# erget/libaec

Measured on AMD Instinct MI355X. Metric: encode+decode GB/s (input bytes), higher is better.
Workload: dtype u32; 1 GPU; c2: lowent16 4096 MiB per GPU, 16-bit, block 16, rsi 128, flags 8; step = encode + decode (segment table); block_size=16, rsi=128, flags=8, input_bytes_per_gpu=4294967296, compressed_bytes_rank0=763194472, parallelism=1 independent shard stream(s)

## Files before the change

libaec_amd/csrc/aec_dec.hip:

```cpp
#include <hip/hip_runtime.h>

#include <cstdio>
#include <cstdlib>
#include <mutex>
#include <type_traits>

#include "aec_kernels.h"
#include "aec_lane.h"
#include "aec_spec.h"
#include "aec_tune.h"

namespace aec {

struct SegSum {
    int64_t sum, lo, hi;
    uint64_t end;
    uint32_t ref;
    uint32_t ok;
};

struct BareArgs {
    SegSum *sums = nullptr;
    const uint32_t *list = nullptr, *list_cnt = nullptr;
    uint64_t avg_hint = 0;
};

struct DecLaunch {
    const Cfg *c = nullptr;
    const uint32_t *words = nullptr;
    uint64_t nwords = 0, end_bit = 0;
    const uint64_t *rsi_off = nullptr;
    const SegEntry *seg_table = nullptr;
    uint64_t n_items = 0, total_blocks = 0;
    uint8_t *out = nullptr;
    DecResult *res = nullptr;
    hipStream_t st = nullptr;
    uint8_t *dump = nullptr;
    const DecResult *idx = nullptr, *batch = nullptr;
    uint32_t rpc = 0;
    bool win = false;
    bool next_entry = false;
    uint32_t rpc_arg() const { return win ? (next_entry ? 1u : 0u) : rpc; }
    BareArgs ba;
};
template <int BS> void dec_part_bytes(bool seg, bool sums, const DecLaunch &a);
template <int BS> void dec_part_wave(const DecLaunch &a);

namespace {

__device__ __forceinline__ uint32_t wave_incl_sum_dpp(uint32_t v)
{
    v += __builtin_amdgcn_update_dpp(0u, v, 0x111, 0xf, 0xf, false);
    v += __builtin_amdgcn_update_dpp(0u, v, 0x112, 0xf, 0xf, false);
    v += __builtin_amdgcn_update_dpp(0u, v, 0x114, 0xf, 0xf, false);
    v += __builtin_amdgcn_update_dpp(0u, v, 0x118, 0xf, 0xf, false);
    v += __builtin_amdgcn_update_dpp(0u, v, 0x142, 0xa, 0xf, false);
    v += __builtin_amdgcn_update_dpp(0u, v, 0x143, 0xc, 0xf, false);
    return v;
}

template <int BS, int BYTES>
__device__ __forceinline__ void store_block(uint8_t *dst, const uint32_t *d, const Cfg &c, bool ref,
                                            uint32_t &x)
{
    const bool pp = c.flags & F_PREPROCESS, sgn = c.flags & F_SIGNED, msb = c.flags & F_MSB;
    uint32_t v[BS];
    if (!pp) {
#pragma unroll
        for (int i = 0; i < BS; i++) v[i] = d[i];
    } else {
        const uint32_t x0 = ref ? (sgn ? sign_extend(d[0], c.bps) : d[0]) : x;
        const uint32_t d0 = ref ? 0u : d[0];
        uint32_t sum = d0, any = 0;
#pragma unroll
        for (int i = 1; i + 1 < BS; i += 2) sum += d[i] + d[i + 1];
        if (BS % 2 == 0) sum += d[BS - 1];
        if (BYTES == 4) {
#pragma unroll
            for (int i = 0; i < BS; i++) any |= i == 0 ? d0 : d[i];
        }
        const uint32_t below = sgn ? x0 + c.xmax + 1u : x0, above = c.xmax - x0;
        const bool fits = sum <= below && sum <= above && (BYTES != 4 || (any >> 26) == 0u);
        if (!__any(!fits)) {
            uint32_t xx = x0;
#pragma unroll
            for (int i = 0; i < BS; i++) {
                const uint32_t di = i == 0 ? d0 : d[i];
                xx += (di >> 1) ^ (uint32_t)__builtin_amdgcn_sbfe((int)di, 0u, 1u);
                v[i] = xx;
            }
            x = xx;
        } else {
#pragma unroll
            for (int i = 0; i < BS; i++) {
                if (i == 0 && ref) {
                    x = x0;
                } else {
                    x = sgn ? unpp_signed(x, d[i], c.xmax) : unpp_unsigned(x, d[i], c.xmax);
                }
                v[i] = x;
            }
        }
    }
    if (BYTES == 4) {
        uint4 *o = reinterpret_cast<uint4 *>(dst);
#pragma unroll
        for (int q = 0; q < BS / 4; q++) {
            uint32_t w[4];
#pragma unroll
            for (int j = 0; j < 4; j++) w[j] = msb ? bswap32(v[4 * q + j]) : v[4 * q + j];
            o[q] = make_uint4(w[0], w[1], w[2], w[3]);
        }
    } else if (BYTES == 2) {
        const uint32_t sel = msb ? 0x04050001u : 0x05040100u;
        uint32_t w[BS / 2];
#pragma unroll
        for (int j = 0; j < BS / 2; j++) w[j] = __builtin_amdgcn_perm(v[2 * j + 1], v[2 * j], sel);
        if (BS >= 8) {
            uint4 *o = reinterpret_cast<uint4 *>(dst);
#pragma unroll
            for (int q = 0; q < BS / 8; q++) o[q] = make_uint4(w[4 * q], w[4 * q + 1], w[4 * q + 2], w[4 * q + 3]);
        }
    } else if (BYTES == 1) {
        uint32_t w[BS / 4];
#pragma unroll
        for (int j = 0; j < BS / 4; j++)
            w[j] = __builtin_amdgcn_perm(v[4 * j + 1], v[4 * j], 0x0c0c0400u) |
                   __builtin_amdgcn_perm(v[4 * j + 3], v[4 * j + 2], 0x04000c0cu);
        uint2 *o = reinterpret_cast<uint2 *>(dst);
#pragma unroll
        for (int q = 0; q < BS / 8; q++) o[q] = make_uint2(w[2 * q], w[2 * q + 1]);
    } else {
#pragma unroll
        for (int i = 0; i < BS; i++) {
            const uint32_t s = v[i];
            dst[3 * i + 0] = (uint8_t)(msb ? s >> 16 : s);
            dst[3 * i + 1] = (uint8_t)(s >> 8);
            dst[3 * i + 2] = (uint8_t)(msb ? s : s >> 16);
        }
    }
}

__device__ __forceinline__ void store_block_generic(uint8_t *dst, const uint32_t *d, const Cfg &c, bool ref,
                                                    uint32_t &x)
{
    const bool pp = c.flags & F_PREPROCESS, sgn = c.flags & F_SIGNED, msb = c.flags & F_MSB;
    for (uint32_t i = 0; i < c.bs; i++) {
        uint32_t v;
        if (!pp) v = d[i];
        else if (i == 0 && ref) v = x = sgn ? sign_extend(d[0], c.bps) : d[0];
        else v = x = sgn ? unpp_signed(x, d[i], c.xmax) : unpp_unsigned(x, d[i], c.xmax);
        for (uint32_t t = 0; t < c.bytes; t++)
            dst[i * c.bytes + t] = (uint8_t)(v >> (8 * (msb ? c.bytes - 1 - t : t)));
    }
}

__device__ __forceinline__ void report(DecResult *res, uint32_t status, uint64_t rsi, uint64_t block)
{
    atomicMax(&res->status, status);
    atomicMin(reinterpret_cast<unsigned long long *>(&res->bad_rsi), (unsigned long long)rsi);
    atomicMin(reinterpret_cast<unsigned long long *>(&res->tail_blocks), (unsigned long long)block);
}

template <bool SEG>
__device__ __forceinline__ void dec_counts(const Cfg &c, const DecResult *idx, uint64_t &n_items, uint64_t &total_blocks)
{
    if (!idx) return;
    const uint64_t whole = idx->n_rsi, tail = idx->tail_blocks;
    n_items = whole + (tail ? 1u : 0u);
    total_blocks = whole * c.rsi + tail;
    if (SEG) n_items *= c.segs_per_rsi;
}

struct DecItem {
    uint32_t nb;
    uint64_t start, first_blk;
};
__device__ __forceinline__ DecItem dec_item(const Cfg &c, uint64_t r, uint64_t total_blocks, const uint64_t *__restrict__ rsi_off,
                                            const DecResult *__restrict__ batch, uint32_t rsi_per_chunk)
{
    DecItem it;
    if (batch) {
        const uint64_t sidx = r / rsi_per_chunk;
        const uint32_t rin = (uint32_t)(r - sidx * rsi_per_chunk);
        const uint64_t whole = batch[sidx].n_rsi, tail = batch[sidx].tail_blocks;
        it.nb = rin < whole ? c.rsi : (rin == whole ? (uint32_t)tail : 0u);
        it.start = it.nb ? rsi_off[r] : 0;
    } else {
        const uint64_t left = total_blocks - r * c.rsi;
        it.nb = left > c.rsi ? c.rsi : (uint32_t)left;
        it.start = rsi_off[r];
    }
    it.first_blk = r * c.rsi;
    return it;
}

__device__ __forceinline__ void report_item(DecResult *res, const DecResult *batch, uint32_t rsi_per_chunk, uint32_t status,
                                            uint64_t r, uint64_t block)
{
    report(res, status, r, block);
    if (batch && status == DEC_DATA_ERROR)
        atomicMax(&const_cast<DecResult *>(batch)[r / rsi_per_chunk].status, (uint32_t)DEC_DATA_ERROR);
}

__device__ __forceinline__ void win_end_check(const Cfg &c, DecResult *res, const uint64_t *__restrict__ rsi_off, uint64_t r,
                                              uint64_t n_rsi, uint32_t next_entry, uint64_t end, uint64_t last_blk)
{
    if (r + 1u < n_rsi + next_entry) {
        const uint64_t e = (c.flags & F_PAD_RSI) ? (end + 7u) & ~7ull : end;
        if (e != rsi_off[r + 1u]) report(res, DEC_DATA_ERROR, r, last_blk);
    }
}

struct RingSrc {
    const uint32_t *col;
    uint32_t slot0, mask;
    uint32_t limit;
    uint32_t starve;
    __device__ __forceinline__ uint32_t word(uint32_t i)
    {
        starve |= (i >= limit) ? 1u : 0u;
        return col[((slot0 + i) & mask) * 64u];
    }
    __device__ __forceinline__ void word2(uint32_t i, uint32_t &w0, uint32_t &w1)
    {
        starve |= (i + 1 >= limit) ? 1u : 0u;
        const uint32_t *q = col + ((slot0 + i) & mask) * 64u;
        w0 = q[0];
        w1 = q[64];
    }
    __device__ __forceinline__ void word3(uint32_t i, uint32_t &w0, uint32_t &w1, uint32_t &w2)
    {
        starve |= (i + 2 >= limit) ? 1u : 0u;
        const uint32_t *q = col + ((slot0 + i) & mask) * 64u;
        w0 = q[0];
        w1 = q[64];
        w2 = q[128];
    }
    __device__ __forceinline__ bool starved() const { return starve != 0; }
};

__device__ __forceinline__ uint4 load_words4(const uint32_t *__restrict__ words, uint64_t idx, uint64_t nwords)
{
    uint4 v = make_uint4(0, 0, 0, 0);
    if (idx + 4 <= nwords) {
        v = *reinterpret_cast<const uint4 *>(words + idx);
    } else {
        if (idx < nwords) v.x = words[idx];
        if (idx + 1 < nwords) v.y = words[idx + 1];
        if (idx + 2 < nwords) v.z = words[idx + 2];
    }
    return v;
}

__device__ __forceinline__ uint4 load_words4_nb(const uint32_t *__restrict__ words, uint64_t idx, uint64_t last_chunk)
{
    if (idx > last_chunk) idx = last_chunk;
    return *reinterpret_cast<const uint4 *>(words + idx);
}

__device__ __forceinline__ void ring_put4(uint32_t *col, uint32_t slot0, uint32_t mask, uint32_t rel, uint4 v)
{
    const uint32_t row = (slot0 + rel) & mask;
    uint32_t *q = col + row * 64u;
    const uint32_t x = bswap32(v.x), y = bswap32(v.y);
    q[0] = x;
    q[64] = y;
    q[128] = bswap32(v.z);
    q[192] = bswap32(v.w);
    if (row == 0) {
        col[(mask + 1u) * 64u] = x;
        col[(mask + 2u) * 64u] = y;
    }
}

template <int BYTES>
struct SumAcc {
    typedef int64_t type;
    static constexpr int64_t kLo = -((int64_t)1 << 60), kHi = (int64_t)1 << 60;
};
template <>
struct SumAcc<1> {
    typedef int32_t type;
    static constexpr int32_t kLo = -(1 << 30), kHi = 1 << 30;
};
template <>
struct SumAcc<2> {
    typedef int32_t type;
    static constexpr int32_t kLo = -(1 << 30), kHi = 1 << 30;
};

template <int BS, typename ACC>
__device__ __forceinline__ void seg_accumulate(const uint32_t *d, bool first_is_ref, ACC R, ACC &P, ACC &lo, ACC &hi)
{
#pragma unroll
    for (int i = 0; i < BS; i++) {
        const uint32_t v = (i == 0 && first_is_ref) ? 0u : d[i];
        const ACC h = (ACC)((v >> 1) + (v & 1u));
        const ACC step = (v & 1u) ? -h : h;
        const ACC nlo = h - P, nhi = R - h - P;
        lo = nlo > lo ? nlo : lo;
        hi = nhi < hi ? nhi : hi;
        P += step;
    }
}

#ifndef AEC_STG_ROW
#define AEC_STG_ROW 64
#endif
#ifndef AEC_STG_ROW8
#define AEC_STG_ROW8 32
#endif
#ifndef AEC_DEC_MINW
#define AEC_DEC_MINW 1
#endif
#ifndef AEC_DEC_UNR8
#define AEC_DEC_UNR8 2
#endif
#ifndef AEC_DEC_OU
#define AEC_DEC_OU 1
#endif
#ifndef AEC_DEC_UNR16
#define AEC_DEC_UNR16 1
#endif
__host__ __device__ constexpr uint32_t dec_unroll(int bs) { return bs == 8 ? AEC_DEC_UNR8 : (bs == 16 ? AEC_DEC_UNR16 : 1); }
__host__ __device__ constexpr bool stg_on(int blk) { return blk == 16 || blk == 32 || (blk == 8 && AEC_STG_ROW8 != 0); }
__host__ __device__ constexpr uint32_t stg_row(int blk) { return blk == 8 ? (AEC_STG_ROW8 ? AEC_STG_ROW8 : 64) : AEC_STG_ROW; }

template <int BS, int BYTES, bool SEG, int kPend, bool SUMS = false, bool WIN = false>
__global__ void __launch_bounds__(256, AEC_DEC_MINW)
k_decode(const Cfg c, const uint32_t *__restrict__ words, uint64_t nwords, uint64_t end_bit,
         const uint64_t *__restrict__ rsi_off, const SegEntry *__restrict__ seg_table, uint64_t n_rsi,
         uint64_t total_blocks, uint8_t *__restrict__ out, DecResult *res, uint32_t ring_words, uint32_t maxw,
         uint32_t needw, uint8_t *__restrict__ dump, const DecResult *__restrict__ idx,
         const DecResult *__restrict__ batch, uint32_t rsi_per_chunk, SegSum *__restrict__ sums,
         const uint32_t *__restrict__ list, const uint32_t *__restrict__ list_cnt)
{
    static_assert(!SUMS || (SEG && BS != 0), "the summing pass runs per segment on the templated block sizes");
    static_assert(!WIN || (!SEG && !SUMS), "windows are tables of RSI starts");
    if (idx) {
        const uint64_t whole = idx->n_rsi, tail = idx->tail_blocks;
        n_rsi = whole + (tail ? 1u : 0u);
        total_blocks = whole * c.rsi + tail;
        if (SEG) n_rsi *= c.segs_per_rsi;
    }
    extern __shared__ __attribute__((aligned(16))) uint32_t smem[];
    const uint32_t lane = threadIdx.x & 63u, wave = threadIdx.x >> 6;
    const uint64_t nwords_vec = nwords >= 4 ? ((nwords + 3) & ~3ull) - 4 : 0;
    constexpr int BLK = BS * BYTES;
    constexpr bool STG = !SUMS && stg_on(BLK);
    constexpr uint32_t kStgRow = stg_row(BLK), kStgStride = kStgRow + 16u;
    constexpr uint32_t G = STG ? kStgRow / (uint32_t)(BLK ? BLK : 1) : 1u;
    const uint32_t wave_words = (ring_words + 2u) * 64u + (STG ? (64u * kStgStride) / 4u : 0u);
    uint32_t *wbase = smem + (size_t)wave * wave_words;
    uint32_t *col = wbase + lane;
    uint8_t *stage = reinterpret_cast<uint8_t *>(wbase + (ring_words + 2u) * 64u);
    const uint32_t mask = ring_words - 1;

    uint64_t r = ((uint64_t)blockIdx.x * (blockDim.x >> 6) + wave) * 64u + lane;
    bool active = r < n_rsi;
    if (!SEG && list) {
        active = r < *list_cnt;
        r = active ? list[r] : 0u;
    }
    constexpr int DN = BS ? BS : (int)kMaxBlockSize;
    const uint32_t bs = BS ? (uint32_t)BS : c.bs;
    const bool pp = c.flags & F_PREPROCESS;

    uint32_t nb = 0, b0 = 0, x = 0;
    uint64_t start = 0, first_blk = 0;
    if (active) {
        if (SEG) {
            const uint64_t rsi_idx = (r >> 32) ? r / c.segs_per_rsi : (uint64_t)((uint32_t)r / c.segs_per_rsi);
            b0 = (uint32_t)(r - rsi_idx * c.segs_per_rsi) * 64u;
            uint64_t left = total_blocks > rsi_idx * c.rsi ? total_blocks - rsi_idx * c.rsi : 0u;
            if (left > c.rsi) left = c.rsi;
            nb = left <= b0 ? 0u : (left - b0 > 64 ? 64u : (uint32_t)(left - b0));
            if (SUMS) {
                start = rsi_off[r];
            } else {
                const SegEntry e = seg_table[r];
                start = e.bit;
                x = (c.flags & F_SIGNED) ? sign_extend(e.prev, c.bps) : e.prev;
            }
            if (start == ~0ull) {
                start = 0;
                nb = 0;
            }
            first_blk = rsi_idx * c.rsi + b0;
        } else if (batch) {
            const uint64_t sidx = r / rsi_per_chunk;
            const uint32_t rin = (uint32_t)(r - sidx * rsi_per_chunk);
            const uint64_t whole = batch[sidx].n_rsi, tail = batch[sidx].tail_blocks;
            nb = rin < whole ? c.rsi : (rin == whole ? (uint32_t)tail : 0u);
            start = nb ? rsi_off[r] : 0;
            first_blk = r * c.rsi;
        } else {
            uint64_t left = total_blocks - r * c.rsi;
            nb = left > c.rsi ? c.rsi : (uint32_t)left;
            start = rsi_off[r];
            first_blk = r * c.rsi;
        }
    }
    const size_t blk_bytes = (size_t)bs * c.bytes;
    uint8_t *dst = out + (size_t)first_blk * blk_bytes;
    const uint32_t dst_lo = (uint32_t)reinterpret_cast<uintptr_t>(dst), dst_hi = (uint32_t)(reinterpret_cast<uintptr_t>(dst) >> 32);
    uint32_t produced = 0;
    auto flush = [&](uint32_t group) {
        const uint32_t filled = produced * (uint32_t)BLK;
        produced = 0;
        constexpr uint32_t LPR = kStgRow / 16u, RPI = 64u / LPR;
#pragma unroll
        for (uint32_t k = 0; k < LPR; k++) {
            const uint32_t row = k * RPI + lane / LPR, chunk = (lane % LPR) * 16u;
            const uint4 v = *reinterpret_cast<const uint4 *>(stage + row * kStgStride + chunk);
            const uint32_t have = __shfl(filled, (int)row);
            const uintptr_t rbase = (uintptr_t)__shfl(dst_lo, (int)row) | ((uintptr_t)__shfl(dst_hi, (int)row) << 32);
            uint8_t *at = reinterpret_cast<uint8_t *>(rbase) + (size_t)group * kStgRow + chunk;
            uint8_t *q = chunk + 16u <= have ? at : dump + (size_t)lane * 16u;
            typedef uint32_t u32x4 __attribute__((ext_vector_type(4)));
            typedef __attribute__((address_space(1))) u32x4 global_u32x4;
            const u32x4 vv = {v.x, v.y, v.z, v.w};
            if (kStgRow >= 64u)
                __builtin_nontemporal_store(vv, reinterpret_cast<global_u32x4 *>(reinterpret_cast<uintptr_t>(q)));
            else
                *reinterpret_cast<global_u32x4 *>(reinterpret_cast<uintptr_t>(q)) = vv;
            if (BLK == 8) {
                const bool half = have == chunk + 8u;
                if (__any(half)) {
                    typedef uint32_t u32x2 __attribute__((ext_vector_type(2)));
                    typedef __attribute__((address_space(1))) u32x2 global_u32x2;
                    const u32x2 hv = {v.x, v.y};
                    if (half) *reinterpret_cast<global_u32x2 *>(reinterpret_cast<uintptr_t>(at)) = hv;
                }
            }
        }
    };

    const uint64_t a0 = (start >> 5) & ~3ull;
    const uint32_t slot0 = (uint32_t)a0 & mask;
    uint32_t landed = 0;
    for (; landed < ring_words; landed += 4)
        ring_put4(col, slot0, mask, landed, load_words4(words, a0 + landed, nwords));

    RingSrc src{col, slot0, mask, landed, 0u};
    const uint64_t left_bits = end_bit - a0 * 32u;
    const uint32_t end_p = left_bits > 0xFFFFFFF0ull ? 0xFFFFFFF0u : (uint32_t)left_bits;
    uint32_t p = (uint32_t)(start - a0 * 32u);
    WinReader<RingSrc> br;
    if (BS == 0) br.init(src, a0 * 32u, end_bit, p);

    uint4 pend[kPend];
    uint32_t pv[kPend];
#pragma unroll
    for (int j = 0; j < kPend; j++) { pend[j] = make_uint4(0, 0, 0, 0); pv[j] = 0u; }

    uint32_t d[DN];
    uint32_t zrun = 0;
    uint32_t ok = 1u;
    typedef typename SumAcc<BYTES>::type acc_t;
    const acc_t acc_R = (acc_t)(((uint64_t)1 << c.bps) - 1u);
    acc_t acc_P = 0, acc_lo = SumAcc<BYTES>::kLo, acc_hi = SumAcc<BYTES>::kHi;
    uint32_t sum_ref = 0, sum_bad = 0, sum_done = 0;

    constexpr uint32_t UNR = (STG && G % dec_unroll(BS) != 0) ? 1u : dec_unroll(BS);
    constexpr uint32_t OU = (STG && AEC_DEC_OU && G > UNR) ? G / UNR : 1u;
    static_assert(!STG || G % UNR == 0, "a staging row holds whole top-up groups");
    uint32_t b = 0;
    for (; __any(b < nb && ok); b += OU * UNR) {
#pragma unroll
      for (uint32_t ou = 0; ou < OU; ou++) {
        const uint32_t bo = b + ou * UNR;
        const bool live = bo < nb && ok;
        {
            const uint32_t next = BS ? (p >> 5) : br.next;
            if (__any(live && landed - next < needw)) {
#pragma unroll
                for (int j = 0; j < kPend; j++) {
                    if (pv[j]) {
                        ring_put4(col, slot0, mask, landed, pend[j]);
                        landed += 4;
                    }
                    pv[j] = 0u;
                }
                while (__any(live && landed - next < needw)) {
                    uint4 t[kPend];
#pragma unroll
                    for (int j = 0; j < kPend; j++) t[j] = load_words4(words, a0 + landed + 4u * j, nwords);
#pragma unroll
                    for (int j = 0; j < kPend; j++)
                        if (live && landed - next < needw && landed + 4u - next <= ring_words) {
                            ring_put4(col, slot0, mask, landed, t[j]);
                            landed += 4;
                        }
                }
            }
        }

        const uint32_t ref = (pp && b0 + bo == 0) ? 1u : 0u;
        if (BS) {
#pragma unroll
          for (uint32_t uu = 0; uu < UNR; uu++) {
            const uint32_t bb = bo + uu;
            const bool live = bb < nb && ok;
            const uint32_t ref = (pp && b0 + bb == 0) ? 1u : 0u;
            src.limit = landed;
            src.starve = 0u;
            uint32_t nz = 0;
            const bool parse = live && zrun == 0;
            const uint32_t p_save = p;
            uint32_t st;
#pragma nounroll
            for (uint32_t attempt = 0;; attempt++) {
                st = decode_block<(BS ? BS : 2)>(src, p, end_p, d, c, ref, b0 + bb, parse, nz);
                if (attempt != 0 || needw >= maxw || !__any(parse && src.starved())) break;
                const uint32_t first = p_save >> 5;
#pragma unroll
                for (int j = 0; j < kPend; j++) {
                    if (pv[j]) {
                        ring_put4(col, slot0, mask, landed, pend[j]);
                        landed += 4;
                    }
                    pv[j] = 0u;
                }
                while (__any(live && landed + 4u - first <= ring_words)) {
                    if (live && landed + 4u - first <= ring_words) {
                        ring_put4(col, slot0, mask, landed, load_words4(words, a0 + landed, nwords));
                        landed += 4;
                    }
                }
                src.limit = landed;
                src.starve = 0;
                p = p_save;
                nz = 0;
            }
            const bool over = parse && (((p + 31u) >> 5) > landed || (st != DEC_OK && src.starved()));
            if (SUMS) {
                if (parse && (over || st != DEC_OK)) {
                    sum_bad = 1u;
                    ok = 0u;
                } else if (parse && nz) {
                    zrun = nz;
                }
            } else if (over) {
                atomicOr(&res->pad, kDecRedo);
                ok = 0u;
            } else if (parse) {
                if (st != DEC_OK) {
                    report(res, st, SEG ? (first_blk + bb) / c.rsi : r, first_blk + bb);
                    if (batch && st == DEC_DATA_ERROR)
                        atomicMax(&const_cast<DecResult *>(batch)[r / rsi_per_chunk].status, (uint32_t)DEC_DATA_ERROR);
                    ok = 0u;
                } else if (nz) {
                    zrun = nz;
                }
            }
            if (uu == 0) {
#pragma unroll
                for (int j = 0; j < kPend; j++)
                    if (pv[j]) {
                        ring_put4(col, slot0, mask, landed, pend[j]);
                        landed += 4;
                    }
                const uint32_t next = p >> 5;
#pragma unroll
                for (int j = 0; j < kPend; j++) {
                    pv[j] = (live && ok && (landed + 4u * j + 4u - next <= ring_words)) ? 1u : 0u;
                    const uint64_t idx = pv[j] ? a0 + landed + 4u * j : 0;
                    pend[j] = load_words4_nb(words, idx, nwords_vec);
                }
            }
            if (SUMS) {
                const bool st_ok = live && ok;
                const bool rf = ref != 0 && parse;
                if (st_ok) {
                    if (rf) sum_ref = d[0];
                    if (c.flags & F_PREPROCESS) seg_accumulate<DN, acc_t>(d, rf, acc_R, acc_P, acc_lo, acc_hi);
                    sum_done++;
                }
                zrun -= (st_ok && zrun) ? 1u : 0u;
            } else if (STG) {
                const bool st_ok = live && ok;
                store_block<DN, (BYTES ? BYTES : 1)>(stage + lane * kStgStride + (bb % G) * (uint32_t)BLK, d, c,
                                                     ref != 0 && parse, x);
                produced += st_ok ? 1u : 0u;
                zrun -= (st_ok && zrun) ? 1u : 0u;
                if (OU * UNR == G ? (ou * UNR + uu == G - 1u) : ((bb % G) == G - 1u)) flush(bb / G);
            } else {
                const bool st_ok = live && ok;
                uint8_t *q = st_ok ? dst : dump + (size_t)lane * blk_bytes;
                store_block<DN, (BYTES ? BYTES : 1)>(q, d, c, ref != 0 && parse, x);
                dst += st_ok ? blk_bytes : 0;
                zrun -= (st_ok && zrun) ? 1u : 0u;
            }
          }
        } else if (live) {
            br.src.limit = landed;
            bool rf = ref != 0;
            if (zrun == 0) {
                uint32_t nz = 0;
                const uint32_t st = parse_cds<0>(br, d, c, ref, b0 + bo, nz);
                if (br.src.starved()) {
                    atomicOr(&res->pad, kDecRedo);
                    ok = 0u;
                } else if (st != DEC_OK) {
                    report(res, st, r, first_blk + bo);
                    if (batch && st == DEC_DATA_ERROR)
                        atomicMax(&const_cast<DecResult *>(batch)[r / rsi_per_chunk].status, (uint32_t)DEC_DATA_ERROR);
                    ok = 0u;
                } else if (nz) {
                    const uint32_t keep = d[0];
                    for (int i = 0; i < DN; i++) d[i] = 0;
                    if (rf) d[0] = keep;
                    zrun = nz - 1;
                }
            } else {
                zrun--;
                rf = false;
            }
            if (ok) {
                store_block_generic(dst, d, c, rf, x);
                dst += blk_bytes;
                if (rf) d[0] = 0;
            }
        }
    }
    }
    if (STG && (b % G) != 0) flush(b / G);
    if (SUMS) {
        if (active) {
            SegSum o;
            o.sum = (int64_t)acc_P;
            o.lo = (int64_t)acc_lo;
            o.hi = (int64_t)acc_hi;
            o.end = a0 * 32u + p;
            o.ref = sum_ref;
            o.ok = (nb != 0u && !sum_bad && sum_done == nb && zrun == 0u) ? 1u : 0u;
            sums[r] = o;
        }
        return;
    }
    if constexpr (WIN) {
        if (active && ok && nb == c.rsi && r + 1u < n_rsi + rsi_per_chunk) {
            uint64_t e;
            if constexpr (BS != 0) e = a0 * 32u + p;
            else e = br.pos();
            if (c.flags & F_PAD_RSI) e = (e + 7u) & ~7ull;
            if (e != rsi_off[r + 1u]) report(res, DEC_DATA_ERROR, r, first_blk + nb - 1u);
        }
    }
    if (!SEG && active && (list ? first_blk + nb == total_blocks : r + 1 == n_rsi)) res->end_bit = x;
    if (SEG && active && nb && first_blk + nb == total_blocks) res->end_bit = x;
}

template <bool SEG, bool WIN = false>
__global__ void __launch_bounds__(64)
k_decode_redo(const Cfg c, const uint32_t *__restrict__ words, uint64_t nwords, uint64_t end_bit,
              const uint64_t *__restrict__ rsi_off, const SegEntry *__restrict__ seg_table, uint64_t n_rsi,
              uint64_t total_blocks, uint8_t *__restrict__ out, DecResult *res, const DecResult *__restrict__ idx,
              const DecResult *__restrict__ batch, uint32_t rsi_per_chunk, const uint32_t *__restrict__ list,
              const uint32_t *__restrict__ list_cnt)
{
    if (!(*reinterpret_cast<volatile uint32_t *>(&res->pad) & kDecRedo)) return;
    dec_counts<SEG>(c, idx, n_rsi, total_blocks);
    if (!SEG && list) n_rsi = *list_cnt;
    const bool pp = c.flags & F_PREPROCESS;
    const size_t blk_bytes = (size_t)c.bs * c.bytes;
    for (uint64_t r_lin = (uint64_t)blockIdx.x * 64u + threadIdx.x; r_lin < n_rsi; r_lin += (uint64_t)gridDim.x * 64u) {
        const uint64_t r = (!SEG && list) ? list[r_lin] : r_lin;
        uint32_t nb = 0, b0 = 0, x = 0;
        uint64_t start = 0, first_blk = 0;
        if (SEG) {
            const uint64_t rsi_idx = r / c.segs_per_rsi;
            b0 = (uint32_t)(r - rsi_idx * c.segs_per_rsi) * 64u;
            uint64_t left = total_blocks > rsi_idx * c.rsi ? total_blocks - rsi_idx * c.rsi : 0u;
            if (left > c.rsi) left = c.rsi;
            nb = left <= b0 ? 0u : (left - b0 > 64 ? 64u : (uint32_t)(left - b0));
            const SegEntry e = seg_table[r];
            if (e.bit == ~0ull) continue;
            start = e.bit;
            x = (c.flags & F_SIGNED) ? sign_extend(e.prev, c.bps) : e.prev;
            first_blk = rsi_idx * c.rsi + b0;
        } else if (batch) {
            const uint64_t sidx = r / rsi_per_chunk;
            const uint32_t rin = (uint32_t)(r - sidx * rsi_per_chunk);
            const uint64_t whole = batch[sidx].n_rsi, tail = batch[sidx].tail_blocks;
            nb = rin < whole ? c.rsi : (rin == whole ? (uint32_t)tail : 0u);
            start = nb ? rsi_off[r] : 0;
            first_blk = r * c.rsi;
        } else {
            const uint64_t left = total_blocks - r * c.rsi;
            nb = left > c.rsi ? c.rsi : (uint32_t)left;
            start = rsi_off[r];
            first_blk = r * c.rsi;
        }
        uint8_t *dst = out + (size_t)first_blk * blk_bytes;
        BitReader br;
        br.init(words, nwords, end_bit, start);
        uint32_t d[kMaxBlockSize];
        uint32_t zrun = 0;
        bool whole = true;
        for (uint32_t bo = 0; bo < nb; bo++) {
            bool rf = pp && b0 + bo == 0;
            if (zrun == 0) {
                uint32_t nz = 0;
                const uint32_t st = parse_cds<0>(br, d, c, rf ? 1u : 0u, b0 + bo, nz);
                if (st != DEC_OK) {
                    report(res, st, r, first_blk + bo);
                    if (batch && st == DEC_DATA_ERROR)
                        atomicMax(&const_cast<DecResult *>(batch)[r / rsi_per_chunk].status, (uint32_t)DEC_DATA_ERROR);
                    whole = false;
                    break;
                }
                if (nz) {
                    const uint32_t keep = d[0];
                    for (uint32_t i = 0; i < kMaxBlockSize; i++) d[i] = 0;
                    if (rf) d[0] = keep;
                    zrun = nz - 1;
                }
            } else {
                zrun--;
                rf = false;
            }
            store_block_generic(dst, d, c, rf, x);
            dst += blk_bytes;
            if (rf) d[0] = 0;
        }
        if constexpr (WIN) {
            if (whole && nb == c.rsi) win_end_check(c, res, rsi_off, r, n_rsi, rsi_per_chunk, br.pos, first_blk + nb - 1u);
        }
        if (!SEG && (list ? first_blk + nb == total_blocks : r + 1 == n_rsi)) res->end_bit = x;
        if (SEG && nb && first_blk + nb == total_blocks) res->end_bit = x;
    }
}

constexpr uint32_t kDwWin = 1024;
constexpr uint32_t kDwPad = 72;
// ... 390 lines not shown
            for (int i = 0; i < BS; i++) {
                const uint32_t v = (i == 0 && ref_l) ? 0u : d[i];
                ssum += (v >> 1) ^ (0u - (v & 1u));
            }
            if (!act) ssum = 0;
            const uint32_t incl = wave_incl_sum_dpp(ssum);
            const uint32_t has_ref = (uint32_t)__builtin_amdgcn_readlane((int)ref_l, 0);
            const uint32_t refv = (uint32_t)__builtin_amdgcn_readlane((int)d[0], 0);
            const uint32_t xb = has_ref ? (sgn ? sign_extend(refv, c.bps) : refv) : xcarry;
            uint32_t xin = xb + incl - ssum;
            uint32_t xout;
            for (;;) {
                xout = xin;
                store_block<BS, BYTES>(q, d, c, ref_l != 0u, xout);
                const uint32_t prev = (uint32_t)__shfl_up((int)xout, 1);
                const uint64_t wrong = __ballot(act && lane != 0u && !ref_l && prev != xin);
                if (!wrong) break;
                const uint32_t f = (uint32_t)__builtin_ctzll(wrong);
                const uint32_t delta = rdlane(prev - xin, f);
                if (lane >= f) xin += delta;
            }
            if (good) xcarry = rdlane(xout, good - 1u);
            x = xcarry;
        }
        done_blocks += good;
        DW_T1(4);
        if (bad || fail_lane < 64u) break;
    }
    if constexpr (WIN) {
        if (lane == 0 && done_blocks == nb && nb == c.rsi)
            win_end_check(c, res, rsi_off, r, n_rsi, rsi_per_chunk, pos, first_blk + nb - 1u);
    }
    if (lane == 0 && r + 1 == n_rsi) res->end_bit = pp ? xcarry : 0u;
}

#ifndef AEC_DEC_PART
__global__ void __launch_bounds__(64)
k_decode_partial(const Cfg c, const uint32_t *__restrict__ words, uint64_t nwords, uint64_t end_bit,
                 const DecResult *__restrict__ idx, uint8_t *__restrict__ out, DecResult *res)
{
    if (threadIdx.x != 0 || blockIdx.x != 0) return;
    if (idx->pad != 1u || idx->status != DEC_OK) return;
    const uint32_t bs = c.bs, bps = c.bps;
    const bool pp = c.flags & F_PREPROCESS, sgn = c.flags & F_SIGNED, msb = c.flags & F_MSB;
    const uint32_t b = (uint32_t)idx->tail_blocks;
    const uint32_t ref = (pp && b == 0) ? 1u : 0u;
    const uint32_t redo_flag = res->pad & kDecRedo;
    BitReader r;
    r.init(words, nwords, end_bit, idx->end_bit);
    auto has = [&](uint32_t n) { return r.pos + n <= end_bit; };
    auto unary_ok = [&](uint32_t &z) { return r.unary(z) && r.pos <= end_bit; };
    uint32_t d[kMaxBlockSize];
    uint32_t cnt = 0;
    do {
        if (!has(c.id_len)) break;
        const uint32_t id = r.get(c.id_len);
        if (id == 0) {
            if (!has(1)) break;
            const uint32_t sel = r.get(1);
            if (ref) {
                if (!has(bps)) break;
                d[cnt++] = r.get(bps);
            }
            if (!sel) break;
            uint32_t i = ref;
            while (i < bs) {
                uint32_t m = 0, sum = 0, second = 0;
                if (!unary_ok(m)) break;
                if (!se_lookup(m, sum, second)) {
                    report(res, DEC_DATA_ERROR, idx->n_rsi, idx->n_rsi * c.rsi + idx->tail_blocks);
                    break;
                }
                if ((i & 1u) == 0) d[cnt++] = sum - second, i++;
                d[cnt++] = second;
                i++;
            }
        } else if (id == (1u << c.id_len) - 1u) {
            while (cnt < bs && has(bps)) d[cnt++] = r.get(bps);
        } else {
            const uint32_t k = id - 1u;
            if (ref) {
                if (!has(bps)) break;
                d[cnt++] = r.get(bps);
            }
            uint32_t fs[kMaxBlockSize];
            const uint32_t n = bs - ref;
            uint32_t got = 0;
            while (got < n && unary_ok(fs[got])) got++;
            if (got < n) break;
            for (uint32_t i = 0; i < n && has(k); i++) d[cnt++] = (fs[i] << k) + (k ? r.get(k) : 0u);
        }
    } while (false);
    if (cnt >= bs) cnt = bs - 1;
    const uint64_t first = (idx->n_rsi * c.rsi + b) * (uint64_t)bs;
    uint32_t x = 0;
    if (pp && !ref && cnt) x = (uint32_t)res->end_bit;
    for (uint32_t i = 0; i < cnt; i++) {
        uint32_t v;
        if (!pp) v = d[i];
        else if (i == 0 && ref) v = x = sgn ? sign_extend(d[0], bps) : d[0];
        else v = x = sgn ? unpp_signed(x, d[i], c.xmax) : unpp_unsigned(x, d[i], c.xmax);
        for (uint32_t t = 0; t < c.bytes; t++)
            out[(first + i) * c.bytes + t] = (uint8_t)(v >> (8 * (msb ? c.bytes - 1 - t : t)));
    }
    res->pad = cnt | redo_flag;
}

__global__ void k_dec_result_init(DecResult *res)
{
    res->n_rsi = 0;
    res->tail_blocks = ~0ull;
    res->end_bit = 0;
    res->status = DEC_OK;
    res->pad = 0;
    res->bad_rsi = ~0ull;
}

uint8_t *dump_buffer()
{
    static std::mutex mu;
    static uint8_t *buf[64] = {};
    int dev = 0;
    (void)hipGetDevice(&dev);
    std::lock_guard<std::mutex> lock(mu);
    if (dev < 0 || dev >= 64) dev = 0;
    if (!buf[dev] && hipMalloc(reinterpret_cast<void **>(&buf[dev]), 64 * kMaxBlockSize * 4) != hipSuccess) {
        buf[dev] = nullptr;
        (void)hipGetLastError();
    }
    return buf[dev];
}
#endif

struct DecGeom {
    uint32_t ring_words, maxw, needw, waves, grid;
    size_t lds_bytes;
};

DecGeom dec_geom(const Cfg &c, uint64_t n_rsi, uint64_t avg_cds_bits, uint32_t stg_row_bytes)
{
    DecGeom g;
    const uint32_t maxbits = (c.id_len + 1 + c.bps + c.bs * c.bps) * dec_unroll((int)c.bs);
    g.maxw = maxbits / 32 + 5;
    uint32_t rw = 16;
    while (rw < 2 * g.maxw + 3) rw <<= 1;
    g.needw = g.maxw;
    const uint64_t hf = tune("AEC_DEC_HALF_FACTOR", 2);
    if (rw >= 32 && g.maxw <= rw / 2 - 3 && avg_cds_bits && avg_cds_bits * hf <= (uint64_t)rw / 2 * 32) {
        rw /= 2;
        g.needw = rw / 2;
    }
    g.ring_words = rw;
    const size_t pad = tune("AEC_DEC_LDS_PAD", 0);
    const size_t per_wave = (size_t)(rw + 2) * 64 * 4 + (stg_row_bytes ? 64 * (stg_row_bytes + 16) : 0) + pad;
    uint32_t waves = 1, best = 0;
    for (uint32_t w = 1; w <= 4; w *= 2) {
        if (per_wave * w > 65536) break;
        uint32_t fit = (uint32_t)(160 * 1024 / (per_wave * w)) * w;
        if (fit > 32) fit = 32;
        if (fit >= best) {
            best = fit;
            waves = w;
        }
    }
    g.waves = waves;
    g.lds_bytes = per_wave * waves;
    const uint64_t nwaves = (n_rsi + 63) / 64;
    g.grid = (uint32_t)((nwaves + waves - 1) / waves);
    return g;
}

template <int BS, int BYTES, bool SEG, int KP, bool SUMS, bool WIN>
void go_lanes(const DecLaunch &a, const DecGeom &g)
{
    hipLaunchKernelGGL((k_decode<BS, BYTES, SEG, KP, SUMS, WIN>), dim3(g.grid), dim3(64 * g.waves), g.lds_bytes, a.st, *a.c,
                       a.words, a.nwords, a.end_bit, a.rsi_off, a.seg_table, a.n_items, a.total_blocks, a.out, a.res,
                       g.ring_words, g.maxw, g.needw, a.dump, a.idx, a.batch, a.rpc_arg(), a.ba.sums, a.ba.list, a.ba.list_cnt);
}

template <int BS, int BYTES, bool WIN>
void go_wave(const DecLaunch &a, const DecGeom &g)
{
    hipLaunchKernelGGL((k_decode_wave<BS, BYTES, WIN>), dim3(g.grid), dim3(64 * g.waves), g.lds_bytes, a.st, *a.c, a.words,
                       a.nwords, a.end_bit, a.rsi_off, a.n_items, a.total_blocks, a.out, a.res, a.dump, a.idx, a.batch, a.rpc_arg());
}

template <bool SEG, bool WIN>
void go_redo(const DecLaunch &a, const DecGeom &g)
{
    hipLaunchKernelGGL((k_decode_redo<SEG, WIN>), dim3(g.grid), dim3(64 * g.waves), g.lds_bytes, a.st, *a.c, a.words, a.nwords,
                       a.end_bit, a.rsi_off, a.seg_table, a.n_items, a.total_blocks, a.out, a.res, a.idx, a.batch, a.rpc_arg(),
                       a.ba.list, a.ba.list_cnt);
}

template <class F>
void with_container_bytes(const Cfg &c, F &&f)
{
    switch (c.bytes) {
    case 1: f(std::integral_constant<int, 1>()); break;
    case 2: f(std::integral_constant<int, 2>()); break;
    case 3: f(std::integral_constant<int, 3>()); break;
    default: f(std::integral_constant<int, 4>()); break;
    }
}

template <int BS, bool SEG, bool SUMS>
void launch_lanes(const DecLaunch &a)
{
    const Cfg &c = *a.c;
    [[maybe_unused]] constexpr bool kCanWin = !SEG && !SUMS;
    if constexpr (BS == 0) {
        const DecGeom g = dec_geom(c, a.n_items, 0, 0u);
        if constexpr (kCanWin) {
            if (a.win) return go_lanes<0, 0, false, 2, false, true>(a, g);
        }
        go_lanes<0, 0, SEG, 2, false, false>(a, g);
    } else {
        const uint32_t blk = (uint32_t)BS * c.bytes;
        const uint64_t avg = (a.total_blocks && !a.idx && !a.batch) ? a.end_bit / a.total_blocks : a.ba.avg_hint;
        const DecGeom g = dec_geom(c, a.n_items, avg, (!SUMS && stg_on((int)blk)) ? stg_row((int)blk) : 0u);
        const uint32_t e_kp = tune("AEC_DEC_KP", 0);
        int kp = BS >= 32 ? (avg == 0 || avg > 512 ? 8 : (avg > 256 ? 4 : 2)) : (avg > 256 ? 4 : 2);
        if (e_kp) kp = e_kp >= 8 ? (BS >= 32 ? 8 : 4) : (e_kp >= 4 ? 4 : 2);
        with_container_bytes(c, [&](auto by) {
            constexpr int B = decltype(by)::value;
            if constexpr (kCanWin) {
                if (a.win) return go_lanes<BS, B, false, 4, false, true>(a, g);
            }
            if (kp == 2) go_lanes<BS, B, SEG, 2, SUMS, false>(a, g);
            else if (kp == 4) go_lanes<BS, B, SEG, 4, SUMS, false>(a, g);
            else if constexpr (BS >= 32) go_lanes<BS, B, SEG, 8, SUMS, false>(a, g);
        });
    }
}

}

#ifdef AEC_DEC_PART
template <int BS>
void dec_part_bytes(bool seg, bool sums, const DecLaunch &a)
{
    if constexpr (BS != 0) {
        if (sums) return launch_lanes<BS, true, true>(a);
    }
    if (seg) launch_lanes<BS, true, false>(a);
    else launch_lanes<BS, false, false>(a);
}

template <int BS>
void dec_part_wave(const DecLaunch &a)
{
    const Cfg &c = *a.c;
    DecGeom g = {};
    g.waves = 2;
    g.grid = (uint32_t)((a.n_items + g.waves - 1) / g.waves);
    g.lds_bytes = (size_t)g.waves * dw_wave_words(c) * 4;
#ifdef AEC_TUNING
    static const bool dw_prof = tune("AEC_DW_PROF", 0) != 0;
    if (dw_prof) {
        unsigned long long z[8] = {0, 0, 0, 0, 0, 0, 0, 0};
        (void)hipMemcpyToSymbolAsync(HIP_SYMBOL(g_dw_prof), z, sizeof(z), 0, hipMemcpyHostToDevice, a.st);
    }
#endif
    with_container_bytes(c, [&](auto by) {
        constexpr int B = decltype(by)::value;
        if (a.win) go_wave<BS, B, true>(a, g);
        else go_wave<BS, B, false>(a, g);
    });
#ifdef AEC_TUNING
    if (dw_prof) {
        static int reports = 0;
        if (reports++ < 6) {
            unsigned long long h[8];
            (void)hipStreamSynchronize(a.st);
            (void)hipMemcpyFromSymbol(h, HIP_SYMBOL(g_dw_prof), sizeof(h));
            fprintf(stderr, "k_decode_wave, RSI 0 (s_memtime ticks): refills %llu | pieces %llu | walk incl. those %llu | "
                    "+ decode %llu | + predictor, store %llu\n", h[0], h[1], h[2], h[3], h[4]);
        }
    }
#endif
}

template void dec_part_bytes<AEC_DEC_PART>(bool, bool, const DecLaunch &);
#if AEC_DEC_PART != 0
template void dec_part_wave<AEC_DEC_PART>(const DecLaunch &);
#endif

#else
extern template void dec_part_bytes<0>(bool, bool, const DecLaunch &);
extern template void dec_part_bytes<8>(bool, bool, const DecLaunch &);
extern template void dec_part_bytes<16>(bool, bool, const DecLaunch &);
extern template void dec_part_bytes<32>(bool, bool, const DecLaunch &);
extern template void dec_part_bytes<64>(bool, bool, const DecLaunch &);
extern template void dec_part_wave<8>(const DecLaunch &);
extern template void dec_part_wave<16>(const DecLaunch &);
extern template void dec_part_wave<32>(const DecLaunch &);
extern template void dec_part_wave<64>(const DecLaunch &);

static bool dec_wave_wanted(const Cfg &c, uint64_t n_items)
{
    if (c.bs != 8u && c.bs != 16u && c.bs != 32u && c.bs != 64u) return false;
    const uint32_t most = tune("AEC_DEC_WAVE_MAX", 8192u), least = tune("AEC_DEC_WAVE_RSI", 16u);
    const uint64_t scaled = c.rsi >= 64u && c.rsi < 128u ? (uint64_t)most * 128u / c.rsi : most;
    return c.rsi >= least && n_items <= scaled;
}

static void launch_items(uint32_t bs, bool seg, bool sums, bool wave, const DecLaunch &a)
// ... 216 lines not shown
```

Baseline: 770.1 GB/s.

## Use raw LDS byte addressing for ring and XOR-swizzle unpadded staging rows

```diff
diff --git a/libaec_amd/csrc/aec_dec.hip b/libaec_amd/csrc/aec_dec.hip
--- a/libaec_amd/csrc/aec_dec.hip
+++ b/libaec_amd/csrc/aec_dec.hip
@@ -61,7 +61,7 @@
 
 template <int BS, int BYTES>
 __device__ __forceinline__ void store_block(uint8_t *dst, const uint32_t *d, const Cfg &c, bool ref,
-                                            uint32_t &x)
+                                            uint32_t &x, uint32_t off = 0u)
 {
     const bool pp = c.flags & F_PREPROCESS, sgn = c.flags & F_SIGNED, msb = c.flags & F_MSB;
     uint32_t v[BS];
@@ -103,13 +103,12 @@
         }
     }
     if (BYTES == 4) {
-        uint4 *o = reinterpret_cast<uint4 *>(dst);
 #pragma unroll
         for (int q = 0; q < BS / 4; q++) {
             uint32_t w[4];
 #pragma unroll
             for (int j = 0; j < 4; j++) w[j] = msb ? bswap32(v[4 * q + j]) : v[4 * q + j];
-            o[q] = make_uint4(w[0], w[1], w[2], w[3]);
+            *reinterpret_cast<uint4 *>(dst + (off ^ (16u * q))) = make_uint4(w[0], w[1], w[2], w[3]);
         }
     } else if (BYTES == 2) {
         const uint32_t sel = msb ? 0x04050001u : 0x05040100u;
@@ -117,9 +116,9 @@
 #pragma unroll
         for (int j = 0; j < BS / 2; j++) w[j] = __builtin_amdgcn_perm(v[2 * j + 1], v[2 * j], sel);
         if (BS >= 8) {
-            uint4 *o = reinterpret_cast<uint4 *>(dst);
-#pragma unroll
-            for (int q = 0; q < BS / 8; q++) o[q] = make_uint4(w[4 * q], w[4 * q + 1], w[4 * q + 2], w[4 * q + 3]);
+#pragma unroll
+            for (int q = 0; q < BS / 8; q++)
+                *reinterpret_cast<uint4 *>(dst + (off ^ (16u * q))) = make_uint4(w[4 * q], w[4 * q + 1], w[4 * q + 2], w[4 * q + 3]);
         }
     } else if (BYTES == 1) {
         uint32_t w[BS / 4];
@@ -127,10 +126,10 @@
         for (int j = 0; j < BS / 4; j++)
             w[j] = __builtin_amdgcn_perm(v[4 * j + 1], v[4 * j], 0x0c0c0400u) |
                    __builtin_amdgcn_perm(v[4 * j + 3], v[4 * j + 2], 0x04000c0cu);
-        uint2 *o = reinterpret_cast<uint2 *>(dst);
-#pragma unroll
-        for (int q = 0; q < BS / 8; q++) o[q] = make_uint2(w[2 * q], w[2 * q + 1]);
+#pragma unroll
+        for (int q = 0; q < BS / 8; q++) *reinterpret_cast<uint2 *>(dst + (off ^ (8u * q))) = make_uint2(w[2 * q], w[2 * q + 1]);
     } else {
+        dst += off;
 #pragma unroll
         for (int i = 0; i < BS; i++) {
             const uint32_t s = v[i];
@@ -212,30 +211,36 @@
     }
 }
 
+typedef __attribute__((address_space(3))) uint32_t lds_u32;
+__device__ __forceinline__ uint32_t ring_at(uint32_t colb, uint32_t s0, uint32_t bm, uint32_t i)
+{
+    return ((((i << 8) + s0)) & bm) | colb;
+}
 struct RingSrc {
-    const uint32_t *col;
-    uint32_t slot0, mask;
+    uint32_t colb;
+    uint32_t s0, bm;
     uint32_t limit;
     uint32_t starve;
+    static __device__ __forceinline__ uint32_t ld(uint32_t a) { return *reinterpret_cast<const lds_u32 *>(a); }
     __device__ __forceinline__ uint32_t word(uint32_t i)
     {
         starve |= (i >= limit) ? 1u : 0u;
-        return col[((slot0 + i) & mask) * 64u];
+        return ld(ring_at(colb, s0, bm, i));
     }
     __device__ __forceinline__ void word2(uint32_t i, uint32_t &w0, uint32_t &w1)
     {
         starve |= (i + 1 >= limit) ? 1u : 0u;
-        const uint32_t *q = col + ((slot0 + i) & mask) * 64u;
-        w0 = q[0];
-        w1 = q[64];
+        const uint32_t t = (i << 8) + s0;
+        w0 = ld((t & bm) | colb);
+        w1 = ld(((t + 256u) & bm) | colb);
     }
     __device__ __forceinline__ void word3(uint32_t i, uint32_t &w0, uint32_t &w1, uint32_t &w2)
     {
         starve |= (i + 2 >= limit) ? 1u : 0u;
-        const uint32_t *q = col + ((slot0 + i) & mask) * 64u;
-        w0 = q[0];
-        w1 = q[64];
-        w2 = q[128];
+        const uint32_t t = (i << 8) + s0;
+        w0 = ld((t & bm) | colb);
+        w1 = ld(((t + 256u) & bm) | colb);
+        w2 = ld(((t + 512u) & bm) | colb);
     }
     __device__ __forceinline__ bool starved() const { return starve != 0; }
 };
@@ -259,19 +264,13 @@
     return *reinterpret_cast<const uint4 *>(words + idx);
 }
 
-__device__ __forceinline__ void ring_put4(uint32_t *col, uint32_t slot0, uint32_t mask, uint32_t rel, uint4 v)
-{
-    const uint32_t row = (slot0 + rel) & mask;
-    uint32_t *q = col + row * 64u;
-    const uint32_t x = bswap32(v.x), y = bswap32(v.y);
-    q[0] = x;
-    q[64] = y;
+__device__ __forceinline__ void ring_put4(uint32_t colb, uint32_t s0, uint32_t bm, uint32_t rel, uint4 v)
+{
+    lds_u32 *q = reinterpret_cast<lds_u32 *>(ring_at(colb, s0, bm, rel));
+    q[0] = bswap32(v.x);
+    q[64] = bswap32(v.y);
     q[128] = bswap32(v.z);
     q[192] = bswap32(v.w);
-    if (row == 0) {
-        col[(mask + 1u) * 64u] = x;
-        col[(mask + 2u) * 64u] = y;
-    }
 }
 
 template <int BYTES>
@@ -326,6 +325,8 @@
 __host__ __device__ constexpr uint32_t dec_unroll(int bs) { return bs == 8 ? AEC_DEC_UNR8 : (bs == 16 ? AEC_DEC_UNR16 : 1); }
 __host__ __device__ constexpr bool stg_on(int blk) { return blk == 16 || blk == 32 || (blk == 8 && AEC_STG_ROW8 != 0); }
 __host__ __device__ constexpr uint32_t stg_row(int blk) { return blk == 8 ? (AEC_STG_ROW8 ? AEC_STG_ROW8 : 64) : AEC_STG_ROW; }
+__host__ __device__ constexpr uint32_t stg_stride(uint32_t row_bytes) { return row_bytes == 64u ? 64u : row_bytes + 16u; }
+__host__ __device__ constexpr uint32_t stg_swz(uint32_t row) { return ((row >> 1) & 3u) << 4; }
 
 template <int BS, int BYTES, bool SEG, int kPend, bool SUMS = false, bool WIN = false>
 __global__ void __launch_bounds__(256, AEC_DEC_MINW)
@@ -349,13 +350,15 @@
     const uint64_t nwords_vec = nwords >= 4 ? ((nwords + 3) & ~3ull) - 4 : 0;
     constexpr int BLK = BS * BYTES;
     constexpr bool STG = !SUMS && stg_on(BLK);
-    constexpr uint32_t kStgRow = stg_row(BLK), kStgStride = kStgRow + 16u;
+    constexpr uint32_t kStgRow = stg_row(BLK), kStgStride = stg_stride(kStgRow);
+    constexpr bool SWZ = STG && kStgStride == kStgRow;
+    static_assert(!SWZ || (kStgRow == 64u && (BLK == 16 || BLK == 32) && BYTES != 3), "stg_swz: four chunks, whole blocks");
     constexpr uint32_t G = STG ? kStgRow / (uint32_t)(BLK ? BLK : 1) : 1u;
-    const uint32_t wave_words = (ring_words + 2u) * 64u + (STG ? (64u * kStgStride) / 4u : 0u);
-    uint32_t *wbase = smem + (size_t)wave * wave_words;
-    uint32_t *col = wbase + lane;
-    uint8_t *stage = reinterpret_cast<uint8_t *>(wbase + (ring_words + 2u) * 64u);
-    const uint32_t mask = ring_words - 1;
+    const uint32_t nwaves = blockDim.x >> 6;
+    const uint32_t lds0 = (uint32_t)reinterpret_cast<uintptr_t>((lds_u32 *)smem);
+    const uint32_t colb = lds0 + wave * ring_words * 256u + lane * 4u;
+    const uint32_t bm = (ring_words - 1u) << 8;
+    uint8_t *stage = reinterpret_cast<uint8_t *>(smem + (size_t)nwaves * ring_words * 64u) + (size_t)wave * (64u * kStgStride);
 
     uint64_t r = ((uint64_t)blockIdx.x * (blockDim.x >> 6) + wave) * 64u + lane;
     bool active = r < n_rsi;
@@ -413,7 +416,7 @@
 #pragma unroll
         for (uint32_t k = 0; k < LPR; k++) {
             const uint32_t row = k * RPI + lane / LPR, chunk = (lane % LPR) * 16u;
-            const uint4 v = *reinterpret_cast<const uint4 *>(stage + row * kStgStride + chunk);
+            const uint4 v = *reinterpret_cast<const uint4 *>(stage + row * kStgStride + (SWZ ? chunk ^ stg_swz(row) : chunk));
             const uint32_t have = __shfl(filled, (int)row);
             const uintptr_t rbase = (uintptr_t)__shfl(dst_lo, (int)row) | ((uintptr_t)__shfl(dst_hi, (int)row) << 32);
             uint8_t *at = reinterpret_cast<uint8_t *>(rbase) + (size_t)group * kStgRow + chunk;
@@ -438,12 +441,12 @@
     };
 
     const uint64_t a0 = (start >> 5) & ~3ull;
-    const uint32_t slot0 = (uint32_t)a0 & mask;
+    const uint32_t s0 = (uint32_t)a0 << 8;
     uint32_t landed = 0;
     for (; landed < ring_words; landed += 4)
-        ring_put4(col, slot0, mask, landed, load_words4(words, a0 + landed, nwords));
-
-    RingSrc src{col, slot0, mask, landed, 0u};
+        ring_put4(colb, s0, bm, landed, load_words4(words, a0 + landed, nwords));
+
+    RingSrc src{colb, s0, bm, landed, 0u};
     const uint64_t left_bits = end_bit - a0 * 32u;
     const uint32_t end_p = left_bits > 0xFFFFFFF0ull ? 0xFFFFFFF0u : (uint32_t)left_bits;
     uint32_t p = (uint32_t)(start - a0 * 32u);
@@ -478,7 +481,7 @@
 #pragma unroll
                 for (int j = 0; j < kPend; j++) {
                     if (pv[j]) {
-                        ring_put4(col, slot0, mask, landed, pend[j]);
+                        ring_put4(colb, s0, bm, landed, pend[j]);
                         landed += 4;
                     }
                     pv[j] = 0u;
@@ -490,7 +493,7 @@
 #pragma unroll
                     for (int j = 0; j < kPend; j++)
                         if (live && landed - next < needw && landed + 4u - next <= ring_words) {
-                            ring_put4(col, slot0, mask, landed, t[j]);
+                            ring_put4(colb, s0, bm, landed, t[j]);
                             landed += 4;
                         }
                 }
@@ -518,14 +521,14 @@
 #pragma unroll
                 for (int j = 0; j < kPend; j++) {
                     if (pv[j]) {
-                        ring_put4(col, slot0, mask, landed, pend[j]);
+                        ring_put4(colb, s0, bm, landed, pend[j]);
                         landed += 4;
                     }
                     pv[j] = 0u;
                 }
                 while (__any(live && landed + 4u - first <= ring_words)) {
                     if (live && landed + 4u - first <= ring_words) {
-                        ring_put4(col, slot0, mask, landed, load_words4(words, a0 + landed, nwords));
+                        ring_put4(colb, s0, bm, landed, load_words4(words, a0 + landed, nwords));
                         landed += 4;
                     }
                 }
@@ -559,7 +562,7 @@
 #pragma unroll
                 for (int j = 0; j < kPend; j++)
                     if (pv[j]) {
-                        ring_put4(col, slot0, mask, landed, pend[j]);
+                        ring_put4(colb, s0, bm, landed, pend[j]);
                         landed += 4;
                     }
                 const uint32_t next = p >> 5;
@@ -581,8 +584,9 @@
                 zrun -= (st_ok && zrun) ? 1u : 0u;
             } else if (STG) {
                 const bool st_ok = live && ok;
-                store_block<DN, (BYTES ? BYTES : 1)>(stage + lane * kStgStride + (bb % G) * (uint32_t)BLK, d, c,
-                                                     ref != 0 && parse, x);
+                const uint32_t at = (bb % G) * (uint32_t)BLK;
+                store_block<DN, (BYTES ? BYTES : 1)>(stage + lane * kStgStride, d, c, ref != 0 && parse, x,
+                                                     SWZ ? at ^ stg_swz(lane) : at);
                 produced += st_ok ? 1u : 0u;
                 zrun -= (st_ok && zrun) ? 1u : 0u;
                 if (OU * UNR == G ? (ou * UNR + uu == G - 1u) : ((bb % G) == G - 1u)) flush(bb / G);
@@ -1279,7 +1283,7 @@
     }
     g.ring_words = rw;
     const size_t pad = tune("AEC_DEC_LDS_PAD", 0);
-    const size_t per_wave = (size_t)(rw + 2) * 64 * 4 + (stg_row_bytes ? 64 * (stg_row_bytes + 16) : 0) + pad;
+    const size_t per_wave = (size_t)rw * 64 * 4 + (stg_row_bytes ? 64 * stg_stride(stg_row_bytes) : 0) + pad;
     uint32_t waves = 1, best = 0;
     for (uint32_t w = 1; w <= 4; w *= 2) {
         if (per_wave * w > 65536) break;
```

Result: no change. 768.7 GB/s (-0.2%).
